# bark-simulator/planner-miqp

Measured on AMD Instinct MI355X. Metric: MIQP solves/sec to 1% gap, 2-agent x 20-step x 32-region, higher is better.
Workload: dtype f64

## Files before the change

planner_miqp_amd/csrc/as_onchip.hip:

```cpp
namespace miqp {

#ifdef MIQP_PROFILE
#define ASP_T(var) const long long var = clock64()
#define ASP_ACC(k, t0, t1) asp_[k] += (unsigned long long)((t1) - (t0))
#else
#define ASP_T(var)
#define ASP_ACC(k, t0, t1)
#endif
constexpr int AS_MAXSTEP = 220;
constexpr double AS_VTOL = 1.0e-8;
constexpr double AS_DEP = 1.0e-8;
constexpr int AS_MT = 64;
constexpr int AS_MSTR = AS_MT * (AS_MT + 1) / 2;

__host__ __device__ constexpr bool as_shape_ok(int C, int N) { return (C == 1 || C == 2) && N >= 1 && N <= 2 * OC_NSL; }

template <int C> __device__ inline int as_col(int pq) { return C == 2 ? ((pq & 3) << 2) | (pq >> 2) : ((pq & 1) << 2) | (pq >> 1); }
template <int C> __device__ inline int as_pcol(int q) { return C == 2 ? ((q & 3) << 2) | (q >> 2) : ((q & 3) << 1) | (q >> 2); }
template <int C> struct AsDecode {
  static constexpr bool LANE_BOUNDS = true, ROW_IDENTITY = true, MARKS = true;
  static __device__ int col(int l) { return as_col<C>(oc_pcol<C, true>(l)); }
};

template <int C, int NSL, int GCAP = miqp::OC_GCAP>
__global__ void __launch_bounds__(64, (GCAP > 128 ? 1 : 2)) as_onchip_kernel(DevBuf B) {
  static_assert(C == 1 || C == 2, "a stage of 16 columns holds the chains of up to two cars");
  constexpr bool CM = true;
  constexpr bool BIG = GCAP > 128;
  constexpr int OC_GCAP = GCAP, OC_GSLOTS = OC_GCAP / 64, OC_GCOEF = oc_gcoef_of(OC_GCAP);
  constexpr int NX = 6 * C, NZ = 8 * C, NCH = 2 * C;
  const Layout& Y = B.Y;
  const int tid = threadIdx.x, lg = tid >> 4, lc = tid & 15;
  const int par = lg >> 1, side = lg & 1;
  const double bsgn = side ? -1.0 : 1.0;
  WAVE_DUMP(BIG ? 1 : 4);
  const int* const clist = BIG && B.cls_take ? B.cls_list + (size_t)(B.cls_take - 1) * B.batch_cap : nullptr;
  const int nbatch = clist ? (B.cls_count[B.cls_take - 1] < B.batch_cap ? B.cls_count[B.cls_take - 1] : B.batch_cap) : (*B.batch_count < B.batch_cap ? *B.batch_count : B.batch_cap);
  const int N = Y.N, NSLOT = Y.NSLOT;
  extern __shared__ double lds[];
  char* const L0 = (char*)lds;
  const OcLds LL = oc_lds_layout(N, Y.fixlen, OC_GCAP, !BIG);
  double* const Z = (double*)(L0 + LL.z);
  double* const scr = (double*)(L0 + LL.u);
  double* const V = (double*)(L0 + LL.u);
  unsigned long long* const bkey = (unsigned long long*)(L0 + LL.r);
  const int SPAN = LL.gmeta - LL.u;
  double* const kref = (double*)(L0 + LL.u + SPAN - N * 32);
  double* const kff = kref - N * 4;
  double* const KS = kff - N * 16;
  const int STG_CAP = (SPAN - N * 192) / 8;
  uint4* const gmeta = (uint4*)(L0 + LL.gmeta);
  double* const gcoef = (double*)(L0 + LL.gcoef);
  double* const grhs = (double*)(L0 + LL.grhs);
  double* const Wd = (double*)(L0 + LL.wd);
  int* const sstart = (int*)(L0 + LL.sstart);
  unsigned short* const cand = (unsigned short*)(L0 + LL.cand);
  signed char* const fix = (signed char*)(L0 + LL.fix);
  __shared__ int sh_node;
  __shared__ unsigned long long sh_stat[32];
  if (tid < 32) sh_stat[tid] = 0ull;
  const unsigned long long lt = (1ull << tid) - 1ull;

  const int chunk = B.as_chunk > 0 ? B.as_chunk : 1;
  int run_next = 0, run_end = 0;
  const int quota = BIG ? 0 : B.as_quota; int handed = 0;
#ifdef MIQP_PROFILE
  const unsigned long long wv_c0 = __builtin_amdgcn_s_memtime(), wv_r0 = __builtin_amdgcn_s_memrealtime();
  unsigned long long wv_first = 0; int wv_nodes = 0;
  if (!BIG && tid == 0) wv_first = atomicMin(&B.prof[120], wv_r0);
#endif
  for (;;) {
    __syncthreads();
    if (run_next >= run_end) {
      if (quota > 0 && handed >= quota) break;
      ++handed;
      if (tid == 0) sh_node = atomicAdd(B.work_counter, chunk);
      __syncthreads();
      run_next = __builtin_amdgcn_readfirstlane(sh_node); run_end = run_next + chunk;
      if (run_next >= nbatch) break;
    }
    const int slot_ = run_next++;
    if (slot_ >= nbatch) { run_next = run_end; continue; }
    const int node = clist ? __builtin_amdgcn_readfirstlane(clist[slot_]) : slot_;
    {
      const int cls = B.batch_large ? (int)B.batch_large[node] : (is_probe_word(B.batch_depth[node]) ? 1 : 0);
      if (cls != (BIG ? 1 : 0)) continue;
    }
    WAVE_DUMP_NODE();
    const int inst = __builtin_amdgcn_readfirstlane(B.batch_inst[node]);
    const double* D = B.inst_d + (size_t)inst * Y.dstride;
    const int* T = B.inst_i + (size_t)inst * Y.istride;
// ... 33 lines not shown
    }
    const int NM = sstart[N + 1];
    OC_WAVE_SYNC();

    ASP_T(ta1); ASP_ACC(0, ta0, ta1);
#ifdef MIQP_PROFILE
    asp_[9] += (unsigned long long)(ocd_t_sparse - ta0); asp_[11] += (unsigned long long)(ta1 - ocd_t_rows);
#endif
    double brhs[NSL];
    unsigned int bact = 0u, binA = 0u, ginA = 0u;
#pragma unroll
    for (int k = 0; k < NSL; ++k) {
      const int i = 2 * k + par;
      brhs[k] = 1e300;
      if (i < N && lc < NZ) {
        const unsigned long long key = bkey[(i * 2 + side) * 16 + lc];
        if (key != ~0ull) { brhs[k] = key2d(key); bact |= 1u << k; }
      }
    }
    OC_WAVE_SYNC();

    const double h1 = ts, h2 = 0.5 * ts * ts, h3 = ts * ts * ts / 6.0;
    const double* const tb = D + Y.d_astab;
    if constexpr (C == 2) {
      for (int k = tid; k < N * 16; k += 64) KS[k] = tb[k];
      for (int k = tid; k < N * 4; k += 64) kref[k] = tb[N * 16 + k];
    } else {
      for (int k = tid; k < N * 8; k += 64) KS[(k >> 3) * 16 + (k & 7)] = tb[k];
      for (int k = tid; k < N * 2; k += 64) kref[(k >> 1) * 4 + (k & 1)] = tb[N * 8 + k];
    }
    OC_WAVE_SYNC();
    typedef double d2_t __attribute__((ext_vector_type(2)));
    auto subst = [&](const bool fromx0, const int itop, const int iend, double* const out) {
      for (int k = tid; k < (N - 1) * 4; k += 64) if ((k >> 2) > itop) kff[k] = fromx0 ? kref[k] : 0.0;
      if (tid < NCH) {
        const int ch = tid;
        double p0 = 0.0, p1 = 0.0, p2 = 0.0;
        int i0 = itop;
        if (itop >= N - 1) { const d2_t a = *(const d2_t*)(V + (N - 1) * 16 + 4 * ch); p0 = a[0]; p1 = a[1]; p2 = V[(N - 1) * 16 + 4 * ch + 2]; i0 = N - 2; }
        if (i0 >= 0) {
          d2_t va = *(const d2_t*)(V + i0 * 16 + 4 * ch), vb = *(const d2_t*)(V + i0 * 16 + 4 * ch + 2);
          d2_t ka = *(const d2_t*)(KS + (i0 * 4 + ch) * 4), kb = *(const d2_t*)(KS + (i0 * 4 + ch) * 4 + 2);
          double kr = fromx0 ? kref[i0 * 4 + ch] : 0.0;
          for (int i = i0; i >= 0; --i) {
            const int j = i > 0 ? i - 1 : 0;
            const d2_t nva = *(const d2_t*)(V + j * 16 + 4 * ch), nvb = *(const d2_t*)(V + j * 16 + 4 * ch + 2);
            const d2_t nka = *(const d2_t*)(KS + (j * 4 + ch) * 4), nkb = *(const d2_t*)(KS + (j * 4 + ch) * 4 + 2);
            const double nkr = fromx0 ? kref[j * 4 + ch] : 0.0;
            const double su = vb[1] + h3 * p0 + h2 * p1 + h1 * p2;
            const double sx0 = va[0] + p0, sx1 = va[1] + h1 * p0 + p1, sx2 = vb[0] + h2 * p0 + h1 * p1 + p2;
            kff[i * 4 + ch] = fma(su, kb[1], kr);
            p0 = sx0 - ka[0] * su; p1 = sx1 - ka[1] * su; p2 = sx2 - kb[0] * su;
            va = nva; vb = nvb; ka = nka; kb = nkb; kr = nkr;
          }
        }
      }
      OC_WAVE_SYNC();
      if (tid < NCH) {
        const int ch = tid;
        double x0 = 0.0, x1 = 0.0, x2 = 0.0;
        if (fromx0) { const int c = ch >> 1, s = ch & 1; x0 = D[Y.d_x0 + 6 * c + 3 * s]; x1 = D[Y.d_x0 + 6 * c + 3 * s + 1]; x2 = D[Y.d_x0 + 6 * c + 3 * s + 2]; }
        const int ie = iend < N - 1 ? iend : N - 2;
        d2_t ka = *(const d2_t*)(KS + ch * 4), kb = *(const d2_t*)(KS + ch * 4 + 2);
        double kf = kff[ch];
        for (int i = 0; i <= ie; ++i) {
          const int j = i < N - 2 ? i + 1 : N - 2;
          const d2_t nka = *(const d2_t*)(KS + (j * 4 + ch) * 4), nkb = *(const d2_t*)(KS + (j * 4 + ch) * 4 + 2);
          const double nkf = kff[j * 4 + ch];
          const double u = -kf - (ka[0] * x0 + ka[1] * x1 + kb[0] * x2);
          d2_t oa, ob; oa[0] = x0; oa[1] = x1; ob[0] = x2; ob[1] = u;
          *(d2_t*)(out + i * 16 + 4 * ch) = oa; *(d2_t*)(out + i * 16 + 4 * ch + 2) = ob;
          const double n0 = x0 + h1 * x1 + h2 * x2 + h3 * u, n1 = x1 + h1 * x2 + h2 * u, n2 = x2 + h1 * u;
          x0 = n0; x1 = n1; x2 = n2;
          ka = nka; kb = nkb; kf = nkf;
        }
        if (iend >= N - 1 || ie == N - 2) { d2_t oa, ob; oa[0] = x0; oa[1] = x1; ob[0] = x2; ob[1] = 0.0; *(d2_t*)(out + (ie + 1) * 16 + 4 * ch) = oa; *(d2_t*)(out + (ie + 1) * 16 + 4 * ch + 2) = ob; }
      }
      OC_WAVE_SYNC();
    };
    auto row_dot = [&](int id, const double* vec) -> double {
      if (id < 1024) return (((id >> 4) & 1) ? -1.0 : 1.0) * vec[(id >> 5) * 16 + (id & 15)];
      const uint4 m4 = gmeta[id - 1024];
      const int off = (int)(m4.z & 0xFFFFu), nn = (int)((m4.z >> 16) & 7u), i = (int)((m4.z >> 20) & 0x7FFu);
      double a = 0.0;
#pragma unroll
      for (int k = 0; k < 6; ++k) if (k < nn) a += gcoef[off + k] * vec[i * 16 + ((m4.w >> (4 * k)) & 15u)];
      return a;
    };
    auto row_soft = [&](int id) -> bool { return id >= 1024 && (gmeta[id - 1024].z & 0x80000000u) != 0u; };
    auto zeroV = [&]() { for (int k = tid; k < N * 16; k += 64) V[k] = 0.0; OC_WAVE_SYNC(); };
    auto objective = [&]() -> double {
      double o = 0.0;
      for (int k = tid; k < N * 16; k += 64) { const int q = k & 15; if (q < NZ) { const double d = Z[k] - Rf[(k >> 4) * NZ + oc_lcol<C, CM>(as_pcol<C>(q))]; o += Wd[q] * d * d; } }
      return wave_sum(o);
    };

    int arow = -1, astage = -1; double alam = 0.0, arhs = 0.0;
    double M[64];
#pragma unroll
    for (int b = 0; b < 64; ++b) M[b] = 0.0;
    unsigned long long used = 0ull;
    auto rank1 = [&](const double u, const double alpha, const unsigned long long mask) {
#pragma unroll
      for (int g8 = 0; g8 < 8; ++g8) {
        if ((mask >> (8 * g8)) & 0xFFull) {
#pragma unroll
          for (int j = 0; j < 8; ++j) { const int b = 8 * g8 + j; M[b] = fma(u * readlane_d(u, b), alpha, M[b]); }
        }
      }
    };
    auto refresh = [&]() {
      zeroV();
      const double FX = 274877906944.0, IFX = 1.0 / 274877906944.0;
      if (arow >= 0 && alam != 0.0) {
        if (arow < 1024) atomicAdd((unsigned long long*)&V[(arow >> 5) * 16 + (arow & 15)], (unsigned long long)(long long)__double2ll_rn((((arow >> 4) & 1) ? -alam : alam) * FX));
        else {
          const uint4 m4 = gmeta[arow - 1024];
          const int off = (int)(m4.z & 0xFFFFu), nn = (int)((m4.z >> 16) & 7u), i = (int)((m4.z >> 20) & 0x7FFu);
#pragma unroll
          for (int k = 0; k < 6; ++k) if (k < nn) atomicAdd((unsigned long long*)&V[i * 16 + ((m4.w >> (4 * k)) & 15u)], (unsigned long long)(long long)__double2ll_rn(gcoef[off + k] * alam * FX));
        }
      }
      OC_WAVE_SYNC();
      for (int k = tid; k < N * 16; k += 64) V[k] = (double)(long long)__double_as_longlong(V[k]) * IFX;
      const int amax = (int)wave_max((double)astage);
      OC_WAVE_SYNC();
      subst(true, amax, N - 1, Z);
    };
    if constexpr (C == 2) { for (int k = tid; k < N * 16; k += 64) Z[k] = tb[N * 20 + k]; }
    else { for (int k = tid; k < N * 16; k += 64) Z[k] = (k & 15) < NZ ? tb[N * 10 + (k >> 4) * NZ + (k & 15)] : 0.0; }
    OC_WAVE_SYNC();
    ASP_T(ta2); ASP_ACC(1, ta1, ta2);
    int steps = 0, ndrop = 0, ok = 1, nwarm = 0, nfast = 0, ncold = 0;
    bool infeas = false, fail = false;
    int why = 0;
    if (B.pool_A && (B.batch_depth[node] >> 6) >= 1 && B.batch_node[node] < B.z_cap) {
      const int rec = B.batch_node[node];
      const unsigned int pa = B.pool_A[(size_t)rec * 64 + tid];
      int cid = -1;
      int ownl = 0;
      if (pa < 1024u) ownl = (int)((((pa >> 5) & 1u) * 2u + ((pa >> 4) & 1u)) << 4 | (pa & 15u));
      const unsigned int ob = (unsigned int)__shfl((int)bact, ownl);
      if (pa < 1024u) { if ((ob >> (pa >> 6)) & 1u) cid = (int)pa; }
      else if (pa != 0xFFFFu) {
        const int pc = (int)pa - 1024;
        int lo = 0, hi = NM;
        while (lo < hi) { const int mid = (lo + hi) >> 1; if ((int)cand[mid] < pc) lo = mid + 1; else hi = mid; }
        if (lo < NM && (int)cand[lo] == pc) cid = 1024 + lo;
      }
      const unsigned long long u0p = __ballot(pa != 0xFFFFu);
      const unsigned long long u0 = __ballot(cid >= 0);
      if (u0) {
        arow = cid;
        astage = cid < 0 ? -1 : (cid < 1024 ? (cid >> 5) : (int)((gmeta[cid - 1024].z >> 20) & 0x7FFu));
        int nmp = 0; unsigned long long moff = 0ull;
        if (B.ring_M) {
          const unsigned long long tg = B.pool_Mtag[rec];
          const unsigned long long c_ = tg >> 8;
          if (tg != 0ull && *(volatile unsigned long long*)B.ring_head - c_ < B.ring_doubles - B.ring_margin) { nmp = (int)(tg & 255ull); moff = c_ % B.ring_doubles; }
        }
        nmp = __builtin_amdgcn_readfirstlane(nmp);
        if (B.as_stats && tid == 0 && !(nmp > 0 && nmp == __popcll(u0p))) sh_stat[16 + (B.ring_M == nullptr ? 0 : (B.pool_Mtag[rec] == 0ull ? 1 : (nmp == 0 ? 2 : 3)))] += 1ull;
        if (nmp > 0 && nmp == __popcll(u0p)) {
          const double* const rm = B.ring_M; const unsigned long long rd_ = B.ring_doubles;
          const int ra = __popcll(u0p & lt);
          const bool mine = (u0p >> tid) & 1ull;
          const int len = nmp * (nmp + 1) / 2;
          for (int c0 = 0; c0 < len; c0 += STG_CAP) {
            const int c1 = c0 + STG_CAP < len ? c0 + STG_CAP : len;
            OC_WAVE_SYNC();
            for (int k = c0 + tid; k < c1; k += 64) { unsigned long long q_ = moff + (unsigned long long)k; if (q_ >= rd_) q_ -= rd_; V[k - c0] = rm[q_]; }
            OC_WAVE_SYNC();
#pragma unroll
            for (int b8 = 0; b8 < 64; ++b8) {
              if ((u0p >> b8) & 1ull) {
                const int rb = __popcll(u0p & ((1ull << b8) - 1ull));
                const int hi_ = ra > rb ? ra : rb, lo_ = ra > rb ? rb : ra;
                const int ix = hi_ * (hi_ + 1) / 2 + lo_;
                if (mine && ix >= c0 && ix < c1) M[b8] = V[ix - c0];
              }
            }
          }
          OC_WAVE_SYNC();
          used = u0p;
          for (unsigned long long um = u0p & ~u0; um; um &= um - 1ull) {
            const int kd = __builtin_amdgcn_readfirstlane(__ffsll((long long)um) - 1);
            double m = 0.0;
#pragma unroll
            for (int b = 0; b < 64; ++b) m = (b == kd) ? M[b] : m;
            const double mkk = readlane_d(m, kd);
            if (mkk > 0.0) rank1(m, -1.0 / mkk, used);
#pragma unroll
            for (int b = 0; b < 64; ++b) if (b == kd || tid == kd) M[b] = 0.0;
            used &= ~(1ull << kd);
          }
          nfast = 1;
        } else {
          used = u0;
          const int amax0 = (int)wave_max((double)astage);
          double sdiag = 1.0;
          for (unsigned long long um = u0; um; um &= um - 1ull) {
            const int a = __builtin_amdgcn_readfirstlane(__ffsll((long long)um) - 1);
            const int ida = __builtin_amdgcn_readlane(arow, a);
            zeroV();
            if (ida < 1024) { if (tid == 0) V[(ida >> 5) * 16 + (ida & 15)] = ((ida >> 4) & 1) ? -1.0 : 1.0; }
            else {
              const uint4 m4 = gmeta[ida - 1024];
              const int off = (int)(m4.z & 0xFFFFu), nn = (int)((m4.z >> 16) & 7u), i = (int)((m4.z >> 20) & 0x7FFu);
              if (tid < nn) V[i * 16 + ((m4.w >> (4 * tid)) & 15u)] = gcoef[off + tid];
            }
            const int sta = __builtin_amdgcn_readlane(astage, a);
            OC_WAVE_SYNC();
            subst(false, sta, amax0, V);
            double sv = arow >= 0 ? -row_dot(arow, V) : 0.0;
            if (tid == a && row_soft(ida)) sv += iaq;
            if (tid == a) sdiag = sv;
#pragma unroll
            for (int b = 0; b < 64; ++b) M[b] = (b == a) ? sv : M[b];
          }
          for (unsigned long long um = u0; um; um &= um - 1ull) {
            const int k = __builtin_amdgcn_readfirstlane(__ffsll((long long)um) - 1);
            double m = 0.0;
#pragma unroll
            for (int b = 0; b < 64; ++b) m = (b == k) ? M[b] : m;
            const double d = readlane_d(m, k);
            if (!(d > AS_DEP * readlane_d(sdiag, k))) {
#pragma unroll
              for (int b = 0; b < 64; ++b) if (b == k || tid == k) M[b] = 0.0;
              if (tid == k) { arow = -1; astage = -1; }
              used &= ~(1ull << k);
              continue;
            }
            const double invd = 1.0 / d;
#pragma unroll
            for (int g8 = 0; g8 < 8; ++g8) {
              if ((u0 >> (8 * g8)) & 0xFFull) {
#pragma unroll
                for (int j = 0; j < 8; ++j) { const int b = 8 * g8 + j; const double mb = readlane_d(m, b); M[b] = (tid == k) ? M[b] * invd : fma(m * mb, -invd, M[b]); }
              }
            }
#pragma unroll
            for (int b = 0; b < 64; ++b) M[b] = (b == k) ? ((tid == k) ? -invd : m * invd) : M[b];
          }
#pragma unroll
          for (int b = 0; b < 64; ++b) M[b] = (arow < 0) ? 0.0 : -M[b];
        }
        {
          int ol = 0, ok_ = -1;
          if (arow >= 0 && arow < 1024) { ol = (((arow >> 5) & 1) * 2 + ((arow >> 4) & 1)) << 4 | (arow & 15); ok_ = arow >> 6; }
          double rsel = arow >= 1024 ? grhs[arow - 1024] : 0.0;
#pragma unroll
          for (int k = 0; k < NSL; ++k) {
            const double rk = __shfl(brhs[k], ol);
            if (ok_ == k) rsel = rk;
          }
          arhs = rsel;
        }
        double cv = arow >= 0 ? row_dot(arow, Z) - arhs : 0.0;
        for (int guard = 0; guard < 64; ++guard) {
          double l0 = 0.0;
#pragma unroll
          for (int g8 = 0; g8 < 8; ++g8) {
            if ((used >> (8 * g8)) & 0xFFull) {
#pragma unroll
              for (int j = 0; j < 8; ++j) { const int b = 8 * g8 + j; l0 = fma(M[b], readlane_d(cv, b), l0); }
            }
          }
          if (arow < 0) l0 = 0.0;
          alam = l0;
          const double lmin = wave_min(arow >= 0 ? l0 : 1e300);
          if (!(lmin < -1e-10)) break;
          const int kd = __builtin_amdgcn_readfirstlane(__ffsll((long long)__ballot(arow >= 0 && l0 == lmin)) - 1);
          double m = 0.0;
#pragma unroll
          for (int b = 0; b < 64; ++b) m = (b == kd) ? M[b] : m;
          const double mkk = readlane_d(m, kd);
          if (!(mkk > 0.0)) { fail = true; break; }
          rank1(m, -1.0 / mkk, used);
#pragma unroll
          for (int b = 0; b < 64; ++b) if (b == kd || tid == kd) M[b] = 0.0;
          if (tid == kd) { arow = -1; astage = -1; alam = 0.0; cv = 0.0; }
          used &= ~(1ull << kd);
          ndrop++;
        }
        if (alam < 0.0) alam = 0.0;
        nwarm = __popcll(used);
        refresh();
        double resid = arow >= 0 ? fabs(row_dot(arow, Z) - arhs - ((arow >= 1024 && row_soft(arow)) ? alam * iaq : 0.0)) : 0.0;
        resid = wave_max(resid);
        if (!(resid <= 1e-7) || fail) {
          fail = false;
          arow = -1; astage = -1; alam = 0.0; arhs = 0.0; used = 0ull; nwarm = 0; nfast = 0; ncold = 1;
#pragma unroll
          for (int b = 0; b < 64; ++b) M[b] = 0.0;
          refresh();
        } else {
          unsigned int* const inab = C == 2 ? (unsigned int*)fix : (unsigned int*)V;
          inab[tid] = 0u;
          OC_WAVE_SYNC();
          if (arow >= 0) {
            if (arow < 1024) atomicOr(&inab[(((arow >> 5) & 1) * 2 + ((arow >> 4) & 1)) << 4 | (arow & 15)], 1u << (arow >> 6));
            else { const int rr_ = arow - 1024; atomicOr(&inab[rr_ & 63], 1u << (16 + (rr_ >> 6))); }
          }
          OC_WAVE_SYNC();
          { const unsigned int w_ = inab[tid]; binA = w_ & 0xFFFFu; ginA = w_ >> 16; }
        }
      }
    }
    ASP_T(ta3); ASP_ACC(8, ta2, ta3);
    double Dval = objective() + wave_sum((arow >= 1024 && row_soft(arow)) ? 0.5 * alam * alam * iaq : 0.0);

    for (; !fail;) {
      ASP_T(tb0);
      double bv = -1e300, brh = 0.0; int bid = -1;
#pragma unroll
      for (int k = 0; k < NSL; ++k) {
        const int i = 2 * k + par;
        if (((bact >> k) & 1u) && !((binA >> k) & 1u)) { const double v = bsgn * Z[i * 16 + lc] - brhs[k]; if (v > bv) { bv = v; brh = brhs[k]; bid = (i * 2 + side) * 16 + lc; } }
      }
#pragma unroll
      for (int q = 0; q < OC_GSLOTS; ++q) {
        const int r = q * 64 + tid;
        if (r < NM && !((ginA >> q) & 1u)) { const double rh_ = grhs[r]; const double v = row_dot(1024 + r, Z) - rh_; if (v > bv) { bv = v; brh = rh_; bid = 1024 + r; } }
      }
      const double vmax = wave_max(bv);
      if (!(vmax > AS_VTOL)) break;
      if (steps >= AS_MAXSTEP || used == ~0ull || !(vmax < 1e290)) { fail = true; why = used == ~0ull ? 1 : 2; break; }
      const int src = __builtin_amdgcn_readfirstlane(__ffsll((long long)__ballot(bv == vmax)) - 1);
      const int pid = __builtin_amdgcn_readlane(bid, src);
      const bool psoft = row_soft(pid);
      const double prhs = readlane_d(brh, src);
      ASP_T(tb1); ASP_ACC(2, tb0, tb1);
      zeroV();
      if (pid < 1024) { if (tid == 0) V[(pid >> 5) * 16 + (pid & 15)] = ((pid >> 4) & 1) ? -1.0 : 1.0; }
      else {
        const uint4 m4 = gmeta[pid - 1024];
        const int off = (int)(m4.z & 0xFFFFu), nn = (int)((m4.z >> 16) & 7u), i = (int)((m4.z >> 20) & 0x7FFu);
        if (tid < nn) V[i * 16 + ((m4.w >> (4 * tid)) & 15u)] = gcoef[off + tid];
      }
      const int pstage = pid < 1024 ? (pid >> 5) : (int)((gmeta[pid - 1024].z >> 20) & 0x7FFu);
      const int amax_ = (int)wave_max((double)astage);
      OC_WAVE_SYNC();
      subst(false, pstage, amax_ > pstage ? amax_ : pstage, V);
      ASP_T(tb2); ASP_ACC(3, tb1, tb2);
      double q = arow >= 0 ? -row_dot(arow, V) : 0.0;
      const double Spp = -row_dot(pid, V) + (psoft ? iaq : 0.0);
      double vp = vmax, lp = 0.0;
      steps++;
      ASP_T(tb3); ASP_ACC(4, tb2, tb3);
      for (;;) {
        double r = 0.0;
#pragma unroll
        for (int g8 = 0; g8 < 8; ++g8) {
          if ((used >> (8 * g8)) & 0xFFull) {
#pragma unroll
            for (int j = 0; j < 8; ++j) { const int b = 8 * g8 + j; r = fma(M[b], readlane_d(q, b), r); }
          }
        }
        if (arow < 0) r = 0.0;
        const double curv = Spp - wave_sum(q * r);
        const double ratio = (arow >= 0 && r > 1e-13) ? alam / r : 1e300;
        const double td = wave_min(ratio);
        const int kd = td < 1e299 ? __builtin_amdgcn_readfirstlane(__ffsll((long long)__ballot(ratio == td)) - 1) : -1;
        if (!(curv == curv) || !(Spp > 0.0)) { fail = true; why = 3; break; }
        const bool dep = !(curv > AS_DEP * Spp);
        double t; bool full;
        if (dep) { if (kd < 0) { infeas = true; break; } t = td; full = false; }
        else { const double tp = vp / curv; if (tp <= td) { t = tp; full = true; } else { t = td; full = false; } }
        if (arow >= 0) { alam = fma(-t, r, alam); if (alam < 0.0) alam = 0.0; }
        lp += t;
        Dval += t * (vp - 0.5 * t * (dep ? 0.0 : curv));
        if (lp > RHO_EL) { infeas = true; break; }
        if (full) {
          const int s = __builtin_amdgcn_readfirstlane(__ffsll((long long)~used) - 1);
          double u = arow >= 0 ? r : 0.0;
          if (tid == s) u = -1.0;
          const unsigned long long nmask = used | (1ull << s);
          rank1(u, 1.0 / curv, nmask);
          if (tid == s) { arow = pid; alam = lp; astage = pstage; arhs = prhs; }
          used = nmask;
          if (pid < 1024) { if (tid == ((((pid >> 5) & 1) * 2 + ((pid >> 4) & 1)) << 4 | (pid & 15))) binA |= 1u << (pid >> 6); }
          else { const int rr_ = pid - 1024; if (tid == (rr_ & 63)) ginA |= 1u << (rr_ >> 6); }
          break;
        }
        vp -= t * (dep ? 0.0 : curv);
        const int idk = __builtin_amdgcn_readlane(arow, kd);
        if (idk < 1024) { if (tid == ((((idk >> 5) & 1) * 2 + ((idk >> 4) & 1)) << 4 | (idk & 15))) binA &= ~(1u << (idk >> 6)); }
        else { const int rr_ = idk - 1024; if (tid == (rr_ & 63)) ginA &= ~(1u << (rr_ >> 6)); }
        double m = 0.0;
#pragma unroll
        for (int b = 0; b < 64; ++b) m = (b == kd) ? M[b] : m;
        const double mkk = readlane_d(m, kd);
        if (!(mkk > 0.0)) { fail = true; why = 4; break; }
        rank1(m, -1.0 / mkk, used);
#pragma unroll
        for (int b = 0; b < 64; ++b) if (b == kd || tid == kd) M[b] = 0.0;
        if (tid == kd) { arow = -1; astage = -1; alam = 0.0; q = 0.0; }
        used &= ~(1ull << kd);
        ndrop++; steps++;
        if (steps >= AS_MAXSTEP) { fail = true; why = 2; break; }
      }
      ASP_T(tb4); ASP_ACC(5, tb3, tb4);
      if (infeas || fail) break;
      refresh();
      ASP_T(tb5); ASP_ACC(6, tb4, tb5);
      if (Dval - 1e-9 * fabs(Dval) > cutoff + 1e-9 * fabs(cutoff)) { ok = 2; break; }
    }
    ASP_T(tc0);
    double viol = 0.0, scost = 0.0, lres = 0.0;
    if (!fail && !infeas && ok == 1) {
#pragma unroll
      for (int k = 0; k < NSL; ++k) { const int i = 2 * k + par; if ((bact >> k) & 1u) viol = fmax(viol, bsgn * Z[i * 16 + lc] - brhs[k]); }
#pragma unroll
      for (int q = 0; q < OC_GSLOTS; ++q) { const int r = q * 64 + tid; if (r < NM && !(gmeta[r].z & 0x80000000u)) viol = fmax(viol, row_dot(1024 + r, Z) - grhs[r]); }
      if (arow >= 0) {
        const bool sf = arow >= 1024 && row_soft(arow);
        const double res = row_dot(arow, Z) - arhs - (sf ? alam * iaq : 0.0);
        if (sf) { scost = 0.5 * alam * alam * iaq; viol = fmax(viol, res); }
        lres = alam * res;
      }
      viol = wave_max(viol); scost = wave_sum(scost);
      lres = fabs(wave_sum(lres));
    } else if (infeas) viol = 1.0;
    if (!fail && !infeas && ok == 1 && !(viol <= 5.0e-7)) { fail = true; why = 5; }
    if (BIG && infeas && B.as_probe_first && B.pump_max > 0 && is_probe_word(B.batch_depth[node]) && (cutoff > 1e299 || B.pump_inc)) fail = true;
    if (fail) {
      if (B.batch_A) B.batch_A[(size_t)node * 64 + tid] = 0xFFFFu;
      if (B.ring_M && tid == 0) B.batch_Mtag[node] = 0ull;
      if (tid == 0) { B.batch_ok[node] = 5; B.pool_big[B.batch_node[node]] |= 4; if (B.as_stats) { sh_stat[2] += 1ull; sh_stat[10 + (why < 6 ? why : 5)] += 1ull; } }
      continue;
    }
    const double obj = (infeas || ok == 2) ? Dval : objective() + scost;
    double* Zo = B.batch_Z + (size_t)node * N * NZ;
    for (int k = tid; k < N * 16; k += 64) { const int q = k & 15; if (q < NZ) Zo[(k >> 4) * NZ + oc_lcol<C, CM>(as_pcol<C>(q))] = Z[k]; }
    if (B.batch_A) {
      unsigned short enc = 0xFFFFu;
      if (!fail && !infeas && ok == 1 && arow >= 0) enc = arow < 1024 ? (unsigned short)arow : (unsigned short)(1024 + (int)cand[arow - 1024]);
      B.batch_A[(size_t)node * 64 + tid] = enc;
    }
    if (B.ring_M) {
      const int n_ = __popcll(used);
      unsigned long long tg_ = 0ull;
      OC_WAVE_SYNC();
      if (!fail && !infeas && ok == 1 && n_ >= 1 && n_ <= AS_MT && n_ * (n_ + 1) * 4 <= LL.total) {
        double* const stg = (double*)L0;
        const int ra = __popcll(used & lt);
#pragma unroll
        for (int b8 = 0; b8 < 64; ++b8) {
          if ((used >> b8) & 1ull) {
            const int rb = __popcll(used & ((1ull << b8) - 1ull));
            if (arow >= 0 && ra >= rb) stg[ra * (ra + 1) / 2 + rb] = M[b8];
          }
        }
        const int len = n_ * (n_ + 1) / 2;
        unsigned long long cnt_ = 0ull;
        if (tid == 0) cnt_ = atomicAdd(B.ring_head, (unsigned long long)len);
        cnt_ = ((unsigned long long)(unsigned int)__builtin_amdgcn_readfirstlane((int)(cnt_ >> 32)) << 32) | (unsigned int)__builtin_amdgcn_readfirstlane((int)cnt_);
        tg_ = (cnt_ << 8) | (unsigned long long)n_;
        OC_WAVE_SYNC();
        const unsigned long long o_ = cnt_ % B.ring_doubles, rd_ = B.ring_doubles;
        for (int k = tid; k < len; k += 64) { unsigned long long q_ = o_ + (unsigned long long)k; if (q_ >= rd_) q_ -= rd_; B.ring_M[q_] = stg[k]; }
      }
      if (tid == 0) B.batch_Mtag[node] = tg_;
    }
    if (tid == 0) {
      B.batch_obj[node] = obj; B.batch_viol[node] = viol; B.batch_ok[node] = ok;
      B.batch_bound[node] = lres + 1e-9 * (1.0 + fabs(obj));
      B.batch_it[node] = steps;
      atomicAdd((unsigned long long*)&B.inst_nodes[inst], 1ull);
      atomicAdd((unsigned long long*)&B.inst_iters[inst], (unsigned long long)steps);
#ifdef MIQP_PROFILE
      ++wv_nodes;
      { const long long tc1 = clock64(); asp_[7] += (unsigned long long)(tc1 - tc0);
        for (int q_ = 0; q_ < 9; ++q_) atomicAdd(&B.prof[80 + q_], asp_[q_]);
        atomicAdd(&B.prof[92], asp_[9]); atomicAdd(&B.prof[93], asp_[11]);
        atomicAdd(&B.prof[90], 1ull); atomicAdd(&B.prof[91], (unsigned long long)steps); }
#endif
      if (B.as_stats) {
        sh_stat[0] += 1ull; sh_stat[1] += (unsigned long long)steps; sh_stat[3] += (unsigned long long)ndrop;
        sh_stat[4] += infeas ? 1ull : 0ull; sh_stat[5] += ok == 2 ? 1ull : 0ull; sh_stat[6] += (unsigned long long)__popcll(used); sh_stat[7] += (unsigned long long)nwarm; sh_stat[8] += (unsigned long long)nfast; sh_stat[9] += (unsigned long long)ncold;
        if (BIG) { const int og_ = B.pool_origin ? (int)B.pool_origin[B.batch_node[node]] : 0; sh_stat[20] += 1ull; sh_stat[21] += (unsigned long long)steps; if (og_ == 14) { sh_stat[22] += 1ull; sh_stat[23] += (unsigned long long)steps; }
          sh_stat[24 + (ngen <= 64 ? 0 : ngen <= 96 ? 1 : ngen <= 128 ? 2 : ngen <= 192 ? 3 : 4)] += 1ull; if (is_probe_word(B.batch_depth[node]) && og_ != 14) sh_stat[29] += 1ull; }
      }
    }
  }
  __syncthreads();
  if (B.as_stats && tid < 32 && sh_stat[tid] != 0ull) atomicAdd(&B.as_stats[tid], sh_stat[tid]);
#ifdef MIQP_PROFILE
  if (!BIG && tid == 0) {
    const unsigned long long wv_c1 = __builtin_amdgcn_s_memtime(), wv_r1 = __builtin_amdgcn_s_memrealtime();
    atomicAdd(&B.prof[94], wv_c1 - wv_c0); atomicAdd(&B.prof[95], wv_r1 - wv_r0); atomicAdd(&B.prof[96], 1ull);
    atomicMin(&B.prof[122], wv_r1); atomicMax(&B.prof[121], wv_r1);
    const unsigned long long dl = wv_r0 > wv_first ? wv_r0 - wv_first : 0ull;
    const int hb = dl < 5000 ? 0 : dl < 20000 ? 1 : dl < 50000 ? 2 : dl < 100000 ? 3 : dl < 200000 ? 4 : dl < 400000 ? 5 : dl < 800000 ? 6 : 7;
    atomicAdd(&B.prof[128 + hb], 1ull);
    const int nb = wv_nodes == 0 ? 0 : wv_nodes <= 4 ? 1 : wv_nodes <= 16 ? 2 : wv_nodes <= 32 ? 3 : wv_nodes <= 64 ? 4 : 5;
    atomicAdd(&B.prof[136 + nb], 1ull);
    if (B.prof[125] == 300 && blockIdx.x < 4096) {
      unsigned int hw, xcc;
      asm volatile("s_getreg_b32 %0, hwreg(HW_REG_HW_ID)" : "=s"(hw));
      asm volatile("s_getreg_b32 %0, hwreg(HW_REG_XCC_ID)" : "=s"(xcc));
      unsigned long long* const w = B.prof + 160 + 4 * blockIdx.x;
      w[0] = wv_r0; w[1] = wv_r1; w[2] = ((unsigned long long)xcc << 32) | hw; w[3] = (unsigned long long)wv_nodes;
    }
  }
#endif
}

}
```

planner_miqp_amd/csrc/kernels.hip:

```cpp
#include <hip/hip_runtime.h>

#include "host_inst.hpp"

#ifndef MIQP_RHO
#define MIQP_RHO 1.0e5
#endif

#ifndef MIQP_IPM_WPE
#define MIQP_IPM_WPE 3
#endif

#ifdef MIQP_ABLATE
#define MIQP_ABL (B.abl)
#else
#define MIQP_ABL 0
#endif
namespace miqp {

constexpr double RHO_EL = MIQP_RHO;
constexpr double FEAS_TOL = 1.0e-6;
constexpr double QP_TOL = 1.0e-6;
#ifndef MIQP_T0
#define MIQP_T0 1.0e-3
#endif
// ... 1337 lines not shown
  if (with_jerk) l = fmax(l, fmax(lift1(fmax(s.ux - rt[16], rt[15] - s.ux), X.uu), lift1(fmax(s.uy - rt[18], rt[17] - s.uy), Yd.uu)));
  if (h == 3) return fmax(l, fmax(lift1(fabs(s.vx) - vm, X.vv), lift1(fabs(s.vy) - vm, Yd.vv)));
  l = fmax(l, lift1(rt[0] * s.vx + rt[1] * s.vy, rt[0] * rt[0] * X.vv + rt[1] * rt[1] * Yd.vv));
  l = fmax(l, lift1(rt[2] * s.vx + rt[3] * s.vy, rt[2] * rt[2] * X.vv + rt[3] * rt[3] * Yd.vv));
  const int* hs = T + Y.i_hs + ((c * Y.P + q) * 2 + h) * 2;
  l = fmax(l, lift1(vm - hs[1] * (hs[0] == 0 ? s.vx : s.vy), hs[0] == 0 ? X.vv : Yd.vv));
  { const double rho = rt[4], k2 = rt[6], k3 = rt[7];
    const double gam = k2 * k2 * X.vv + 2.0 * k2 * rho * X.va + rho * rho * X.aa + k3 * k3 * Yd.vv - 2.0 * k3 * Yd.va + Yd.aa;
    l = fmax(l, lift1(s.ay - rho * s.ax - k2 * s.vx - k3 * s.vy - rt[5], gam)); }
  { const double rho = rt[4], k2 = rt[9], k3 = rt[10];
    const double gam = k2 * k2 * X.vv + 2.0 * k2 * rho * X.va + rho * rho * X.aa + k3 * k3 * Yd.vv - 2.0 * k3 * Yd.va + Yd.aa;
    l = fmax(l, lift1(-s.ay + rho * s.ax + k2 * s.vx + k3 * s.vy + rt[8], gam)); }
  return l;
}

__device__ inline void region_lift_parts(const Layout& Y, const double* D, int c, int q, const CarState& s, bool with_jerk, const LiftBlk& X, const LiftBlk& Yd, double& l0, double& lfast) {
  const double* rt = D + Y.d_reg + (c * Y.P + q) * REGSZ;
  l0 = fmax(lift1(fmax(s.ax - rt[12], rt[11] - s.ax), X.aa), lift1(fmax(s.ay - rt[14], rt[13] - s.ay), Yd.aa));
  if (with_jerk) l0 = fmax(l0, fmax(lift1(fmax(s.ux - rt[16], rt[15] - s.ux), X.uu), lift1(fmax(s.uy - rt[18], rt[17] - s.uy), Yd.uu)));
  lfast = fmax(lift1(rt[0] * s.vx + rt[1] * s.vy, rt[0] * rt[0] * X.vv + rt[1] * rt[1] * Yd.vv), lift1(rt[2] * s.vx + rt[3] * s.vy, rt[2] * rt[2] * X.vv + rt[3] * rt[3] * Yd.vv));
  { const double rho = rt[4], k2 = rt[6], k3 = rt[7];
    const double gam = k2 * k2 * X.vv + 2.0 * k2 * rho * X.va + rho * rho * X.aa + k3 * k3 * Yd.vv - 2.0 * k3 * Yd.va + Yd.aa;
    lfast = fmax(lfast, lift1(s.ay - rho * s.ax - k2 * s.vx - k3 * s.vy - rt[5], gam)); }
  { const double rho = rt[4], k2 = rt[9], k3 = rt[10];
    const double gam = k2 * k2 * X.vv + 2.0 * k2 * rho * X.va + rho * rho * X.aa + k3 * k3 * Yd.vv - 2.0 * k3 * Yd.va + Yd.aa;
    lfast = fmax(lfast, lift1(-s.ay + rho * s.ax + k2 * s.vx + k3 * s.vy + rt[8], gam)); }
}
__device__ inline double region_lift_from(const Layout& Y, const double* D, const int* T, int c, int q, int h, const CarState& s, const LiftBlk& X, const LiftBlk& Yd, double l0, double lfast) {
  const double vm = D[Y.d_glob + 6];
  if (h == 3) return fmax(l0, fmax(lift1(fabs(s.vx) - vm, X.vv), lift1(fabs(s.vy) - vm, Yd.vv)));
  const int* hs = T + Y.i_hs + ((c * Y.P + q) * 2 + h) * 2;
  return fmax(fmax(l0, lfast), lift1(vm - hs[1] * (hs[0] == 0 ? s.vx : s.vy), hs[0] == 0 ? X.vv : Yd.vv));
}

struct BranchDesc { int prio; int kind; int c; int o; int i; int pt; int cause; };

#ifndef MIQP_EVAL_WPE
#define MIQP_EVAL_WPE 0
#endif
template <int C>
#if MIQP_EVAL_WPE > 0
__global__ void __launch_bounds__(64, MIQP_EVAL_WPE) eval_kernel(DevBuf B) {
#else
__global__ void __launch_bounds__(64) eval_kernel(DevBuf B) {
#endif
  constexpr int NZ = 8 * C;
  const Layout& Y = B.Y;
  const int node = blockIdx.x, lane = threadIdx.x;
  if (node >= *B.batch_count || node >= B.batch_cap) return;
  if (lane == 0) B.batch_candkey[node] = ~0ull;
#define FREE_NODE() do { if (lane == 0) { unsigned int q_ = atomicAdd(B.free_tail, 1u); B.free_q[q_ % (unsigned int)B.pool_cap] = B.batch_node[node]; } } while (0)
  const int inst = B.batch_inst[node];
  const int slot = B.inst_slot[inst];
  const double* D = B.inst_d + (size_t)inst * Y.dstride;
  const int* T = B.inst_i + (size_t)inst * Y.istride;
  const int N = Y.N, P = Y.P;
  extern __shared__ double lds[];
  double* Z = lds;
  float* slowv = (float*)(Z + N * NZ);
  double* gsc = Z + N * NZ;
  double* fastv = Z + N * NZ + eval_shared_doubles(C, N, P);
  double* rlift = fastv + C * N;
  int* fastc = (int*)(rlift + C * N);
  int* vflag = fastc + C * N;
  int* altbuf = vflag + C * N;
  double* altval = (double*)(altbuf + 64);
  signed char* fix = (signed char*)(altval + 64);
  signed char* comp = fix + Y.fixlen;
  signed char* cfix = comp + Y.fixlen;
  double* mr_g = (double*)(cfix + ((Y.fixlen + 7) & ~7));
  double* mr_y = mr_g + LIFT_ROWS * NZ;
  double* mr_v = mr_y + LIFT_ROWS * NZ;
  double* mr_d = mr_v + LIFT_ROWS;
  double* mr_l = mr_d + LIFT_ROWS;
  double* mr_w = mr_l + LIFT_ROWS;
  signed char* ploose = (B.seq_kinds & 0x80000000u) ? (signed char*)(mr_w + NZ) : (signed char*)mr_g;
  __shared__ BranchDesc chosen;
  __shared__ int sh_base[4];
  __shared__ int slots[64];
  __shared__ int ck[64], ca[64], fam[4];
  __shared__ int k_ck[64], k_ca[64], k_neg[64], k_ord[64], k_pos[64];
  __shared__ double clift[64], k_bnd[64];

  const double* Zi = B.batch_Z + (size_t)node * N * NZ;
  const signed char* src = B.pool_fix + (size_t)B.batch_node[node] * Y.fixlen;
  PROF_T(te0);
  for (int k = lane; k < N * NZ; k += 64) Z[k] = Zi[k];
  for (int k8 = lane; k8 < Y.fixlen / 8; k8 += 64) { const unsigned long long w8 = ((const unsigned long long*)src)[k8]; ((unsigned long long*)fix)[k8] = w8; ((unsigned long long*)comp)[k8] = w8; ((unsigned long long*)ploose)[k8] = 0ull; }
  __syncthreads();
  PROF_T(te1);
  const double viol = B.batch_viol[node];
  const int okq = B.batch_ok[node];
  if (okq == 5) {
    if (lane == 0) {
      const int pos = atomicAdd(&B.open_count[inst], 1);
      if (pos < B.open_cap) { const size_t oi = ((size_t)B.open_sel * B.n_slots + slot) * B.open_cap + pos; B.open_bound[oi] = B.batch_bound[node]; B.open_node[oi] = B.batch_node[node]; B.open_depth[oi] = B.batch_depth[node]; }
      else { atomicOr(&B.inst_flags[inst], 1); unsigned int q_ = atomicAdd(B.free_tail, 1u); B.free_q[q_ % (unsigned int)B.pool_cap] = B.batch_node[node]; }
    }
    return;
  }
  const unsigned char big_parent = B.pool_big ? B.pool_big[B.batch_node[node]] : 0;
  if (B.stats && lane == 0) {
    const int oc_ = okq == 2 ? 1 : (viol > FEAS_TOL ? 0 : (okq != 1 ? 2 : 3));
    atomicAdd(&B.stats[32 + oc_], 1ull); atomicAdd(&B.stats[36 + oc_], (unsigned long long)B.batch_it[node]);
    if (B.pool_origin) { const int og_ = (int)B.pool_origin[B.batch_node[node]] & 15; atomicAdd(&B.stats[80 + og_], 1ull); atomicAdd(&B.stats[96 + 16 * oc_ + og_], 1ull); if (og_ == 15) { const int ib_ = B.batch_it[node] / 3; atomicAdd(&B.stats[192 + 16 * oc_ + (ib_ > 15 ? 15 : ib_)], 1ull); } }
  }
  bool pumped = false;
  if (viol > FEAS_TOL && okq == 1 && B.pump_max > 0 && B.pool_big && is_probe_word(B.batch_depth[node]) && (int)(big_parent >> 4) < B.pump_max
      && (!(fmin(B.live_inc ? inc_from_key(*(volatile unsigned long long*)&B.inc_key[inst]) : B.inc_obj[inst], B.inc_ext[inst]) < 1e300)
          || (B.pump_inc && B.batch_obj[node] + B.inst_const[inst] < fmin(B.inc_obj[inst], B.inc_ext[inst])))) pumped = true;
  if (!pumped && (viol > FEAS_TOL || okq != 1)) { FREE_NODE(); return; }
  if (pumped) {
    for (int k = lane; k < Y.f_rmask + C * N * 2 && k < Y.fixlen; k += 64) { fix[k] = (signed char)-1; comp[k] = (signed char)-1; }
    __syncthreads();
    if (B.stats && lane == 0) atomicAdd(&B.stats[62], 1ull);
  }
  int nign = 0;
  for (int k = lane; k < C * Y.O * N * 5; k += 64) nign += fix[Y.f_obs + k] >= Y.L ? 1 : 0;
  nign = (int)wave_sum((double)nign);
  const double obj = B.batch_obj[node] + B.inst_const[inst] + nign * D[Y.d_misc + 1];
  const double objlb = pumped ? B.lower_bound[inst] : obj - fmax(0.0, B.batch_bound[node]);
  const double inc_now = fmin(B.live_inc ? inc_from_key(*(volatile unsigned long long*)&B.inc_key[inst]) : B.inc_obj[inst], B.inc_ext[inst]);
  if (inc_now < 1e300 && !(objlb < inc_now - 1e-12 * fabs(inc_now))) { if (B.stats && lane == 0) atomicAdd(&B.stats[40], 1ull); FREE_NODE(); return; }
  if (B.stats && lane == 0 && inc_now < 1e300 && (inc_now - objlb) <= B.inst_gap[inst] * (1e-10 + fabs(inc_now))) atomicAdd(&B.stats[41], 1ull);
  const double tol = FEAS_TOL;
  const int NCI = C * (N - 1);
  const double gapi_ = B.inst_gap[inst];
  bool dead_lane = false;
  for (int L0 = 0; L0 < NCI; L0 += 64) {
    int L = L0 + lane;
    if (L < NCI) {
      int c = L / (N - 1), i = 1 + L % (N - 1);
      const double* z = Z + i * NZ;
      CarState s = {z[6 * c], z[6 * c + 1], z[6 * c + 2], z[6 * c + 3], z[6 * c + 4], z[6 * c + 5], z[6 * C + 2 * c], z[6 * C + 2 * c + 1]};
      bool wj = i <= N - 2;
      int np = T[Y.i_nposs + c];
      int nxt = (i + 1 < N) ? (int)fix[Y.f_reg + c * N + i + 1] : -1;
      int nxtq = (nxt >= 0 && (nxt & 3) == 3) ? (nxt >> 2) : -1;
      double bv = 1e300; int bc = -1; bool found = false;
      const bool want_score = ((B.seq_kinds >> 8) & 15) >= 10;
      LiftDiag LX = {0.0, 0.0, 0.0, 0.0}, LYd = {0.0, 0.0, 0.0, 0.0}; if (want_score) lift_diag(Y, D, c, i, LX, LYd);
      double ml = 1e300;
      const unsigned long long allow = ((unsigned long long)(unsigned int)T[Y.i_allow + (c * N + i) * 2 + 1] << 32) | (unsigned int)T[Y.i_allow + (c * N + i) * 2];
      int rset = region_set(Y, T, fix, c, i);
      if (fix[Y.f_reg + c * N + i] < 0 && inc_now < 1e300 && !(B.seq_kinds & 0x8000)) {
        LiftBlk BX, BY; lift_blocks(Y, D, c, i, BX, BY);
        const double room = inc_now - gapi_ * (1e-10 + fabs(inc_now)) - objlb;
        int nleft = 0, last_code = -1;
        for (int q = 0; q < np; ++q) {
          if (!((rset >> q) & 1)) continue;
          if (nxtq >= 0 && nxtq != q) { rset &= ~(1 << q); continue; }
          bool any = false;
          const int nhq = T[Y.i_nhs + c * P + q];
          double bxq, fq, l0q, lfq;
          region_viol_parts(Y, D, c, q, s, wj, bxq, fq); region_lift_parts(Y, D, c, q, s, wj, BX, BY, l0q, lfq);
          for (int h = 0; h < 4; ++h) {
            if ((h < 3 && h >= nhq) || !((allow >> (q * 4 + h)) & 1ull)) continue;
            if (region_lift_from(Y, D, T, c, q, h, s, BX, BY, l0q, lfq) * (1.0 - 1e-6) >= room && region_viol_from(Y, D, T, c, q, h, s, bxq, fq) > tol) continue;
            any = true; nleft++; last_code = q * 4 + h;
          }
          if (!any) rset &= ~(1 << q);
        }
        (void)nleft; (void)last_code;
        if (rset != region_set(Y, T, fix, c, i)) {
          const int idx = Y.f_rmask + 2 * (c * N + i);
          fix[idx] = comp[idx] = (signed char)(rset & 255); fix[idx + 1] = comp[idx + 1] = (signed char)((rset >> 8) & 255);
          if (B.stats) atomicAdd(&B.stats[58], 1ull);
        }
      }
      if (rset == 0 && fix[Y.f_reg + c * N + i] < 0) dead_lane = true;
      for (int q = 0; q < np; ++q) {
        if (nxtq >= 0 && nxtq != q) { slowv[(c * N + i) * P + q] = 3.0e38f; continue; }
        double bxq, fq; region_viol_parts(Y, D, c, q, s, wj, bxq, fq);
        slowv[(c * N + i) * P + q] = !((allow >> (q * 4 + 3)) & 1ull) ? 3.0e38f : (float)fmin(region_viol_from(Y, D, T, c, q, 3, s, bxq, fq), 3.0e38);
        int nh = T[Y.i_nhs + c * P + q];
        for (int h = 0; h < nh; ++h) {
          if (!((allow >> (q * 4 + h)) & 1ull)) continue;
          double v = region_viol_from(Y, D, T, c, q, h, s, bxq, fq);
          if (want_score) ml = fmin(ml, region_alt_lift(Y, D, T, c, q, h, s, wj, LX, LYd));
          if (!found && v <= tol) { found = true; bv = 0.0; bc = q * 4 + h; }
          if (!found && v < bv) { bv = v; bc = q * 4 + h; }
        }
      }
      fastv[c * N + i] = bv; fastc[c * N + i] = bc; vflag[c * N + i] = 0; rlift[c * N + i] = ml < 1e300 ? ml : 0.0;
    }
  }
  __syncthreads();
  PROF_T(te2);
  if (__ballot(dead_lane)) { if (B.stats && lane == 0) atomicAdd(&B.stats[59], 1ull); FREE_NODE(); return; }
  if (lane < C) {
    int c = lane; int prevj = T[Y.i_initj + c];
    int np = T[Y.i_nposs + c];
    for (int i = 1; i < N; ++i) {
      int code = (int)fix[Y.f_reg + c * N + i];
// ... 1261 lines not shown
```

Measured before the change: 1058.

## Cut active-set early on bound, switch-select M columns, defer node loads

```diff
diff --git a/planner_miqp_amd/csrc/as_onchip.hip b/planner_miqp_amd/csrc/as_onchip.hip
--- a/planner_miqp_amd/csrc/as_onchip.hip
+++ b/planner_miqp_amd/csrc/as_onchip.hip
@@ -7,6 +7,8 @@
 #define ASP_T(var)
 #define ASP_ACC(k, t0, t1)
 #endif
+#define AS_SLOTS8(F, o) F((o)) F((o) + 1) F((o) + 2) F((o) + 3) F((o) + 4) F((o) + 5) F((o) + 6) F((o) + 7)
+#define AS_SLOTS64(F) AS_SLOTS8(F, 0) AS_SLOTS8(F, 8) AS_SLOTS8(F, 16) AS_SLOTS8(F, 24) AS_SLOTS8(F, 32) AS_SLOTS8(F, 40) AS_SLOTS8(F, 48) AS_SLOTS8(F, 56)
 constexpr int AS_MAXSTEP = 220;
 constexpr double AS_VTOL = 1.0e-8;
 constexpr double AS_DEP = 1.0e-8;
@@ -206,9 +208,12 @@
       if (id < 1024) return (((id >> 4) & 1) ? -1.0 : 1.0) * vec[(id >> 5) * 16 + (id & 15)];
       const uint4 m4 = gmeta[id - 1024];
       const int off = (int)(m4.z & 0xFFFFu), nn = (int)((m4.z >> 16) & 7u), i = (int)((m4.z >> 20) & 0x7FFu);
+      double c_[6], v_[6];
+#pragma unroll
+      for (int k = 0; k < 6; ++k) { c_[k] = gcoef[off + k]; v_[k] = vec[i * 16 + ((m4.w >> (4 * k)) & 15u)]; }
       double a = 0.0;
 #pragma unroll
-      for (int k = 0; k < 6; ++k) if (k < nn) a += gcoef[off + k] * vec[i * 16 + ((m4.w >> (4 * k)) & 15u)];
+      for (int k = 0; k < 6; ++k) a = k < nn ? fma(c_[k], v_[k], a) : a;
       return a;
     };
     auto row_soft = [&](int id) -> bool { return id >= 1024 && (gmeta[id - 1024].z & 0x80000000u) != 0u; };
@@ -233,6 +238,24 @@
         }
       }
     };
+    auto colM = [&](const int kd_) -> double {
+      const int kd = __builtin_amdgcn_readfirstlane(kd_);
+      double m = 0.0;
+#define AS_PICK(b) case b: m = M[b]; break;
+      switch (kd) { AS_SLOTS64(AS_PICK) default: break; }
+#undef AS_PICK
+      return m;
+    };
+    auto clearM = [&](const int kd_) {
+      const int kd = __builtin_amdgcn_readfirstlane(kd_);
+#define AS_ZERO(b) case b: M[b] = 0.0; break;
+      switch (kd) { AS_SLOTS64(AS_ZERO) default: break; }
+#undef AS_ZERO
+      if (tid == kd) {
+#pragma unroll
+        for (int b = 0; b < 64; ++b) M[b] = 0.0;
+      }
+    };
     auto refresh = [&]() {
       zeroV();
       const double FX = 274877906944.0, IFX = 1.0 / 274877906944.0;
@@ -241,8 +264,11 @@
         else {
           const uint4 m4 = gmeta[arow - 1024];
           const int off = (int)(m4.z & 0xFFFFu), nn = (int)((m4.z >> 16) & 7u), i = (int)((m4.z >> 20) & 0x7FFu);
-#pragma unroll
-          for (int k = 0; k < 6; ++k) if (k < nn) atomicAdd((unsigned long long*)&V[i * 16 + ((m4.w >> (4 * k)) & 15u)], (unsigned long long)(long long)__double2ll_rn(gcoef[off + k] * alam * FX));
+          double c_[6];
+#pragma unroll
+          for (int k = 0; k < 6; ++k) c_[k] = gcoef[off + k];
+#pragma unroll
+          for (int k = 0; k < 6; ++k) if (k < nn) atomicAdd((unsigned long long*)&V[i * 16 + ((m4.w >> (4 * k)) & 15u)], (unsigned long long)(long long)__double2ll_rn(c_[k] * alam * FX));
         }
       }
       OC_WAVE_SYNC();
@@ -255,7 +281,7 @@
     else { for (int k = tid; k < N * 16; k += 64) Z[k] = (k & 15) < NZ ? tb[N * 10 + (k >> 4) * NZ + (k & 15)] : 0.0; }
     OC_WAVE_SYNC();
     ASP_T(ta2); ASP_ACC(1, ta1, ta2);
-    int steps = 0, ndrop = 0, ok = 1, nwarm = 0, nfast = 0, ncold = 0;
+    int steps = 0, ndrop = 0, ok = 1, nwarm = 0, nfast = 0, ncold = 0, ncut = 0;
     bool infeas = false, fail = false;
     int why = 0;
     if (B.pool_A && (B.batch_depth[node] >> 6) >= 1 && B.batch_node[node] < B.z_cap) {
@@ -309,13 +335,10 @@
           used = u0p;
           for (unsigned long long um = u0p & ~u0; um; um &= um - 1ull) {
             const int kd = __builtin_amdgcn_readfirstlane(__ffsll((long long)um) - 1);
-            double m = 0.0;
-#pragma unroll
-            for (int b = 0; b < 64; ++b) m = (b == kd) ? M[b] : m;
+            const double m = colM(kd);
             const double mkk = readlane_d(m, kd);
             if (mkk > 0.0) rank1(m, -1.0 / mkk, used);
-#pragma unroll
-            for (int b = 0; b < 64; ++b) if (b == kd || tid == kd) M[b] = 0.0;
+            clearM(kd);
             used &= ~(1ull << kd);
           }
           nfast = 1;
@@ -344,13 +367,10 @@
           }
           for (unsigned long long um = u0; um; um &= um - 1ull) {
             const int k = __builtin_amdgcn_readfirstlane(__ffsll((long long)um) - 1);
-            double m = 0.0;
-#pragma unroll
-            for (int b = 0; b < 64; ++b) m = (b == k) ? M[b] : m;
+            const double m = colM(k);
             const double d = readlane_d(m, k);
             if (!(d > AS_DEP * readlane_d(sdiag, k))) {
-#pragma unroll
-              for (int b = 0; b < 64; ++b) if (b == k || tid == k) M[b] = 0.0;
+              clearM(k);
               if (tid == k) { arow = -1; astage = -1; }
               used &= ~(1ull << k);
               continue;
@@ -395,14 +415,11 @@
           const double lmin = wave_min(arow >= 0 ? l0 : 1e300);
           if (!(lmin < -1e-10)) break;
           const int kd = __builtin_amdgcn_readfirstlane(__ffsll((long long)__ballot(arow >= 0 && l0 == lmin)) - 1);
-          double m = 0.0;
-#pragma unroll
-          for (int b = 0; b < 64; ++b) m = (b == kd) ? M[b] : m;
+          const double m = colM(kd);
           const double mkk = readlane_d(m, kd);
           if (!(mkk > 0.0)) { fail = true; break; }
           rank1(m, -1.0 / mkk, used);
-#pragma unroll
-          for (int b = 0; b < 64; ++b) if (b == kd || tid == kd) M[b] = 0.0;
+          clearM(kd);
           if (tid == kd) { arow = -1; astage = -1; alam = 0.0; cv = 0.0; }
           used &= ~(1ull << kd);
           ndrop++;
@@ -496,6 +513,7 @@
         Dval += t * (vp - 0.5 * t * (dep ? 0.0 : curv));
         if (lp > RHO_EL) { infeas = true; break; }
         if (full) {
+          if (Dval - 1e-9 * fabs(Dval) > cutoff + 1e-9 * fabs(cutoff)) { ok = 2; ncut = 1; break; }
           const int s = __builtin_amdgcn_readfirstlane(__ffsll((long long)~used) - 1);
           double u = arow >= 0 ? r : 0.0;
           if (tid == s) u = -1.0;
@@ -511,24 +529,20 @@
         const int idk = __builtin_amdgcn_readlane(arow, kd);
         if (idk < 1024) { if (tid == ((((idk >> 5) & 1) * 2 + ((idk >> 4) & 1)) << 4 | (idk & 15))) binA &= ~(1u << (idk >> 6)); }
         else { const int rr_ = idk - 1024; if (tid == (rr_ & 63)) ginA &= ~(1u << (rr_ >> 6)); }
-        double m = 0.0;
-#pragma unroll
-        for (int b = 0; b < 64; ++b) m = (b == kd) ? M[b] : m;
+        const double m = colM(kd);
         const double mkk = readlane_d(m, kd);
         if (!(mkk > 0.0)) { fail = true; why = 4; break; }
         rank1(m, -1.0 / mkk, used);
-#pragma unroll
-        for (int b = 0; b < 64; ++b) if (b == kd || tid == kd) M[b] = 0.0;
+        clearM(kd);
         if (tid == kd) { arow = -1; astage = -1; alam = 0.0; q = 0.0; }
         used &= ~(1ull << kd);
         ndrop++; steps++;
         if (steps >= AS_MAXSTEP) { fail = true; why = 2; break; }
       }
       ASP_T(tb4); ASP_ACC(5, tb3, tb4);
-      if (infeas || fail) break;
+      if (infeas || fail || ok == 2) break;
       refresh();
       ASP_T(tb5); ASP_ACC(6, tb4, tb5);
-      if (Dval - 1e-9 * fabs(Dval) > cutoff + 1e-9 * fabs(cutoff)) { ok = 2; break; }
     }
     ASP_T(tc0);
     double viol = 0.0, scost = 0.0, lres = 0.0;
@@ -556,7 +570,7 @@
     }
     const double obj = (infeas || ok == 2) ? Dval : objective() + scost;
     double* Zo = B.batch_Z + (size_t)node * N * NZ;
-    for (int k = tid; k < N * 16; k += 64) { const int q = k & 15; if (q < NZ) Zo[(k >> 4) * NZ + oc_lcol<C, CM>(as_pcol<C>(q))] = Z[k]; }
+    if (ok != 2) for (int k = tid; k < N * 16; k += 64) { const int q = k & 15; if (q < NZ) Zo[(k >> 4) * NZ + oc_lcol<C, CM>(as_pcol<C>(q))] = Z[k]; }
     if (B.batch_A) {
       unsigned short enc = 0xFFFFu;
       if (!fail && !infeas && ok == 1 && arow >= 0) enc = arow < 1024 ? (unsigned short)arow : (unsigned short)(1024 + (int)cand[arow - 1024]);
@@ -602,7 +616,7 @@
 #endif
       if (B.as_stats) {
         sh_stat[0] += 1ull; sh_stat[1] += (unsigned long long)steps; sh_stat[3] += (unsigned long long)ndrop;
-        sh_stat[4] += infeas ? 1ull : 0ull; sh_stat[5] += ok == 2 ? 1ull : 0ull; sh_stat[6] += (unsigned long long)__popcll(used); sh_stat[7] += (unsigned long long)nwarm; sh_stat[8] += (unsigned long long)nfast; sh_stat[9] += (unsigned long long)ncold;
+        sh_stat[4] += infeas ? 1ull : 0ull; sh_stat[5] += ok == 2 ? 1ull : 0ull; sh_stat[6] += (unsigned long long)(__popcll(used) + ncut); sh_stat[7] += (unsigned long long)nwarm; sh_stat[8] += (unsigned long long)nfast; sh_stat[9] += (unsigned long long)ncold;
         if (BIG) { const int og_ = B.pool_origin ? (int)B.pool_origin[B.batch_node[node]] : 0; sh_stat[20] += 1ull; sh_stat[21] += (unsigned long long)steps; if (og_ == 14) { sh_stat[22] += 1ull; sh_stat[23] += (unsigned long long)steps; }
           sh_stat[24 + (ngen <= 64 ? 0 : ngen <= 96 ? 1 : ngen <= 128 ? 2 : ngen <= 192 ? 3 : 4)] += 1ull; if (is_probe_word(B.batch_depth[node]) && og_ != 14) sh_stat[29] += 1ull; }
       }
@@ -631,4 +645,7 @@
 #endif
 }
 
+#undef AS_SLOTS8
+#undef AS_SLOTS64
+
 }
diff --git a/planner_miqp_amd/csrc/kernels.hip b/planner_miqp_amd/csrc/kernels.hip
--- a/planner_miqp_amd/csrc/kernels.hip
+++ b/planner_miqp_amd/csrc/kernels.hip
@@ -1443,13 +1443,6 @@
   __shared__ int k_ck[64], k_ca[64], k_neg[64], k_ord[64], k_pos[64];
   __shared__ double clift[64], k_bnd[64];
 
-  const double* Zi = B.batch_Z + (size_t)node * N * NZ;
-  const signed char* src = B.pool_fix + (size_t)B.batch_node[node] * Y.fixlen;
-  PROF_T(te0);
-  for (int k = lane; k < N * NZ; k += 64) Z[k] = Zi[k];
-  for (int k8 = lane; k8 < Y.fixlen / 8; k8 += 64) { const unsigned long long w8 = ((const unsigned long long*)src)[k8]; ((unsigned long long*)fix)[k8] = w8; ((unsigned long long*)comp)[k8] = w8; ((unsigned long long*)ploose)[k8] = 0ull; }
-  __syncthreads();
-  PROF_T(te1);
   const double viol = B.batch_viol[node];
   const int okq = B.batch_ok[node];
   if (okq == 5) {
@@ -1471,6 +1464,13 @@
       && (!(fmin(B.live_inc ? inc_from_key(*(volatile unsigned long long*)&B.inc_key[inst]) : B.inc_obj[inst], B.inc_ext[inst]) < 1e300)
           || (B.pump_inc && B.batch_obj[node] + B.inst_const[inst] < fmin(B.inc_obj[inst], B.inc_ext[inst])))) pumped = true;
   if (!pumped && (viol > FEAS_TOL || okq != 1)) { FREE_NODE(); return; }
+  const double* Zi = B.batch_Z + (size_t)node * N * NZ;
+  const signed char* src = B.pool_fix + (size_t)B.batch_node[node] * Y.fixlen;
+  PROF_T(te0);
+  for (int k = lane; k < N * NZ; k += 64) Z[k] = Zi[k];
+  for (int k8 = lane; k8 < Y.fixlen / 8; k8 += 64) { const unsigned long long w8 = ((const unsigned long long*)src)[k8]; ((unsigned long long*)fix)[k8] = w8; ((unsigned long long*)comp)[k8] = w8; ((unsigned long long*)ploose)[k8] = 0ull; }
+  __syncthreads();
+  PROF_T(te1);
   if (pumped) {
     for (int k = lane; k < Y.f_rmask + C * N * 2 && k < Y.fixlen; k += 64) { fix[k] = (signed char)-1; comp[k] = (signed char)-1; }
     __syncthreads();
```

New measurement: 1077 (median of 6 runs). Within noise of the previous version (+1.8%).
